# Woodenonez/DyObAv-MPCnWTA-Warehouse

Hardware: AMD Instinct MI355X
Metric: MPC solves/sec (N=20, batched) (higher is better)
Workload: dtype f32

## Files before the change

### dyobav-mpcnwta-warehouse_amd/csrc/nmpc_device.h

```cpp
#pragma once

#include <hip/hip_runtime.h>

#include "nmpc_sizes.h"
#include "wave_ops.h"

namespace nmpc {

#ifdef NMPC_PROFILE
constexpr int kProfSlots = 16;
#define NMPC_STAMP(I_, slot)                                              \
    do {                                                                  \
        __builtin_amdgcn_sched_barrier(0);                                \
        const unsigned long long t_ = __builtin_amdgcn_s_memtime();       \
        (I_).prof[slot] += t_ - (I_).t_last;                              \
        (I_).t_last = t_;                                                 \
        __builtin_amdgcn_sched_barrier(0);                                \
    } while (0)
#elif defined(NMPC_MARK)
constexpr int kProfSlots = 0;
#define NMPC_STAMP(I_, slot)                                                                      \
    do {                                                                                          \
        __builtin_amdgcn_sched_barrier(0);                                                        \
        if ((slot) < 7 || (slot) > 11) asm volatile("s_nop %0" : : "n"(8 + ((slot) & 7)));   \
// ... 106 lines not shown
__device__ __forceinline__ float tabs(float x) { return fabsf(x); }
__device__ __forceinline__ double tabs(double x) { return fabs(x); }
__device__ __forceinline__ float tpow(float x, float y) { return powf(x, y); }
__device__ __forceinline__ double tpow(double x, double y) { return pow(x, y); }
__device__ __forceinline__ float tmax(float a, float b) { return fmaxf(a, b); }
__device__ __forceinline__ double tmax(double a, double b) { return fmax(a, b); }
__device__ __forceinline__ float tmin(float a, float b) { return fminf(a, b); }
__device__ __forceinline__ double tmin(double a, double b) { return fmin(a, b); }
__device__ __forceinline__ bool tfinite(float x) { return isfinite(x); }
__device__ __forceinline__ bool tfinite(double x) { return isfinite(x); }
__device__ __forceinline__ void sincos_medium(const float x, float& s, float& c)
{
    auto K = [](unsigned bits) { return __builtin_bit_cast(float, bits); };
    const float ax = __builtin_fabsf(x);
    const float fn = __builtin_rintf(ax * K(0x3f22f983u));
    const int n = (int)fn;
    float r = __builtin_fmaf(fn, K(0xbfc90fdau), ax);
    r = __builtin_fmaf(fn, K(0xb3a22168u), r);
    r = __builtin_fmaf(fn, K(0xa7c234c4u), r);
    const float r2 = r * r;
    float t = __builtin_fmaf(r2, K(0xb94c1982u), K(0x3c0881c4u));
    t = __builtin_fmaf(r2, t, K(0xbe2aaa9du));
    t = r2 * t;
    const float sr = __builtin_fmaf(r, t, r);
    float u = __builtin_fmaf(r2, K(0x37d75334u), K(0xbab64f3bu));
    u = __builtin_fmaf(r2, u, K(0x3d2aabf7u));
    u = __builtin_fmaf(r2, u, K(0xbf000004u));
    const float cr = __builtin_fmaf(r2, u, 1.0f);
    const unsigned flip = ((unsigned)n << 30) & 0x80000000u;
    const bool odd = (n & 1) != 0;
    const unsigned sb = __builtin_bit_cast(unsigned, odd ? cr : sr) ^ flip ^
                        (__builtin_bit_cast(unsigned, x) & 0x80000000u);
    const unsigned cb = __builtin_bit_cast(unsigned, odd ? -sr : cr) ^ flip;
    s = __builtin_bit_cast(float, sb);
    c = __builtin_bit_cast(float, cb);
}
constexpr float kSincosMediumBound = 131072.0f;

template <typename T>
__device__ __forceinline__ T tclamp(T x, T lo, T hi)
{
    return tmin(tmax(x, lo), hi);
}
template <typename T>
__device__ __forceinline__ T ls_point(T u, T f, T d, T tau)
{
#pragma clang fp contract(off)
    const T a = (T(1) - tau) * f;
    const T b = tau * d;
    return (u - a) - b;
}

template <typename T>
struct Lim;
template <>
struct Lim<float> {
    static constexpr float min_pos = 1.17549435e-38f, eps = 1.1920929e-7f, big = 3.0e38f;
};
template <>
struct Lim<double> {
    static constexpr double min_pos = 2.2250738585072014e-308, eps = 2.220446049250313e-16, big = 1.0e300;
};

__device__ __forceinline__ double fast_rcp(double x)
{
    x = fmin(x, Lim<double>::big);
    double r = __builtin_amdgcn_rcp(x);
    r = __builtin_fma(__builtin_fma(-x, r, 1.0), r, r);
    r = __builtin_fma(__builtin_fma(-x, r, 1.0), r, r);
    return r;
}
__device__ __forceinline__ float fast_rcp(float x)
{
    x = fminf(x, Lim<float>::big);
    float r = __builtin_amdgcn_rcpf(x);
    r = __builtin_fmaf(__builtin_fmaf(-x, r, 1.0f), r, r);
    return r;
}

template <typename T>
struct alignas(16) Quad {
    T a, b, c, d;
};

template <typename T, int LPS, bool GLB = false, int RS = 0, bool COOP = false, bool HLP = false, bool AXIS = false>
struct Instance {
    static_assert(!AXIS || (RS > 0 && LPS == 3) || GLB, "axis-aligned variant: three-lane register table, or the compressed global table");
    static constexpr bool CMP = AXIS && GLB;
    static_assert(!(GLB && RS > 0), "the register-resident table replaces the LDS table, not the global one");
    static_assert(RS == 0 || LPS == 3 || LPS == 1, "register-resident table: three lanes or one lane per horizon step");
    const KParams<T>& kp;
    const T* __restrict__ p;
    T* lds;
    T* wsp;

    int lane, k, r;
    bool act, lead, tail;

    T rv_k, qstc_k, qdyn_k;

    int n_dyn, n_pad;
    int n_grp = 0;
    int n_poly;
    int n_fl0, n_flp;
    T wzero;

    int n_psi, n_grad;
    int cw_ = 0, CW_ = 1, xb = 0;
    T* coop_x = nullptr;
    __device__ __forceinline__ int cw() const { return COOP ? cw_ : 0; }
    __device__ __forceinline__ int CW() const { return COOP ? CW_ : 1; }
    __device__ __forceinline__ int reg_rows() const { return RS == 0 ? 0 : HLP ? 3 * CW() * (RS / 2) : LPS * CW() * RS; }
    T tab[RS > 0 ? RS : 1][9];
#ifdef NMPC_PROFILE
    unsigned long long* prof;
    unsigned long long t_last;
    unsigned int pcnt[3] = {0u, 0u, 0u};
    __device__ __forceinline__ unsigned long long prof_value(int i) const { return prof[i] + (!COOP && i >= 13 ? pcnt[i - 13] : 0u); }
#endif

    __device__ __forceinline__ Instance(const KParams<T>& kp_, const T* p_, T* lds_, T* ws_ = nullptr)
        : kp(kp_), p(p_), lds(lds_), wsp(ws_)
    {
        lane = threadIdx.x & 63;
        k = lane / LPS;
        r = lane - k * LPS;
        act = k < kp.N;
        lead = act && r == 0;
        tail = act && r == LPS - 1;
        n_psi = n_grad = 0;
#ifdef NMPC_PROFILE
        __shared__ unsigned long long prof_sh[8][kProfSlots];
        prof = prof_sh[(threadIdx.x >> 6) & 7];
        for (int i = 0; i < kProfSlots; ++i) prof[i] = 0;
        t_last = __builtin_amdgcn_s_memtime();
#endif
    }

    __device__ __forceinline__ int load()
    {
        const int N = kp.N, NP1 = kp.N + 1;
        const int kk = act ? k : 0;
        rv_k = p[kp.off_rv + kk];
        qstc_k = p[kp.off_qstc + kk];
        qdyn_k = p[kp.off_qdyn + kk];

        int* iflag = reinterpret_cast<int*>(lds + kp.lds_iflag);
        const unsigned lane_lt = __builtin_amdgcn_mbcnt_hi(~0u, __builtin_amdgcn_mbcnt_lo(~0u, 0u));
        (void)lane_lt;

        const int ne = kp.Ndyn * NP1;
        for (int j = lane; j < kp.Ndyn; j += 64) iflag[j] = 0;
        __syncthreads();
        for (int e = lane; e < ne; e += 64) {
            const T* s = p + kp.off_od + e * 6;
            const bool nz = s[0] != T(0) || s[1] != T(0) || s[2] != T(0) || s[3] != T(0) || s[4] != T(0) ||
                            s[5] != T(0);
            if (nz) iflag[e / NP1] = 1;
        }
        __syncthreads();
        int base = 0;
        for (int j0 = 0; j0 < kp.Ndyn; j0 += 64) {
            const int j = j0 + lane;
            const bool on = j < kp.Ndyn && iflag[j] != 0;
            const unsigned long long bal = __ballot(on);
            const int pos = base + __popcll(bal & ((1ull << lane) - 1ull));
            __syncthreads();
            if (j < kp.Ndyn) iflag[j] = on ? pos : -1;
            base += __popcll(bal);
        }
        n_dyn = base;
        n_pad = kp.Ndyn - base;
        __syncthreads();
        if (n_dyn > kp.dyn_cap) return 4;
        bool skew = false;
        auto offdiag = [](const T x) { return x != T(0) && x == x; };
        auto entry = [&](const T* s, const T marg, Quad<T>& qa, Quad<T>& qb) {
            const T rx = s[2], ry = s[3];
            T sa, ca;
            tsincos(s[4], sa, ca);
            const T exp_ = rx + T(1e-6), eyp = ry + T(1e-6), exm = rx + marg + T(1e-6), eym = ry + marg + T(1e-6);
            const T ixp = T(1) / (exp_ * exp_), iyp = T(1) / (eyp * eyp);
            const T ixm = T(1) / (exm * exm), iym = T(1) / (eym * eym);
            const T cc = ca * ca, ss = sa * sa, cs = ca * sa;
            qa = Quad<T>{s[0], s[1], cc * ixp + ss * iyp, cs * (ixp - iyp)};
            qb = Quad<T>{ss * ixp + cc * iyp, cc * ixm + ss * iym, cs * (ixm - iym), ss * ixm + cc * iym};
        };
        if (RS > 0) {
            int* jof = reinterpret_cast<int*>(lds + kp.lds_hist);
            for (int j = lane; j < kp.Ndyn; j += 64) {
                const int row = iflag[j];
                if (row < 0) continue;
                const T* s = p + kp.off_od + (size_t)j * NP1 * 6;
                Quad<T> qa, qb;
                entry(s, kp.vm + kp.sm, qa, qb);
                Quad<T>* q = reinterpret_cast<Quad<T>*>(lds + row * kEllStride);
// ... 146 lines not shown
            if (i < kp.Nstc) {
#pragma unroll
                for (int c = 0; c < 12; ++c) {
                    v[c] = p[kp.off_os + 12 * i + c];
                    nz = nz || v[c] != T(0);
                }
            }
            const unsigned long long bal = __ballot(nz);
            const int pos = base + __popcll(bal & ((1ull << lane) - 1ull));
            if (nz) {
#pragma unroll
                for (int c = 0; c < 12; ++c) lds[kp.lds_poly + 12 * pos + c] = v[c];
            }
            base += __popcll(bal);
        }
        n_poly = base;
        if (lane < 12 * LPS) lds[kp.lds_poly + 12 * n_poly + lane] = lane % 12 < 4 ? T(-1) : T(0);
        int* idx0 = reinterpret_cast<int*>(lds + kp.lds_fl0);
        int* idxp = reinterpret_cast<int*>(lds + kp.lds_fl);
        int b0 = 0, bp = 0;
        for (int j0 = 0; j0 < kp.Nother; j0 += 64) {
            const int j = j0 + lane;
            bool nz0 = false, nzp = false;
            if (j < kp.Nother) {
                nz0 = j >= 1 && (p[kp.off_c0 + 3 * j] != T(0) || p[kp.off_c0 + 3 * j + 1] != T(0));
                for (int kk = 0; kk < N; ++kk)
                    nzp = nzp || p[kp.off_c + 3 * (j * N + kk)] != T(0) || p[kp.off_c + 3 * (j * N + kk) + 1] != T(0);
            }
            const unsigned long long bal0 = __ballot(nz0), balp = __ballot(nzp);
            const unsigned long long lt = (1ull << lane) - 1ull;
            if (nz0) idx0[b0 + __popcll(bal0 & lt)] = j;
            if (nzp) idxp[bp + __popcll(balp & lt)] = j;
            b0 += __popcll(bal0);
            bp += __popcll(balp);
        }
        n_fl0 = b0;
        n_flp = bp;
        wzero = T(1000) * T(kp.Nother - 1 - b0) + T(10) * T(kp.Nother - bp);
        for (int i = lane; i < N; i += 64) {
            const int i2 = i + 1 < N ? i + 1 : N - 1;
            const T ax = p[kp.off_rs + 3 * i], ay = p[kp.off_rs + 3 * i + 1];
            const T dx = p[kp.off_rs + 3 * i2] - ax, dy = p[kp.off_rs + 3 * i2 + 1] - ay;
            T* q = lds + kp.lds_seg + 4 * i;
            q[0] = ax;
            q[1] = ay;
            q[2] = dx;
            q[3] = dy;
            lds[kp.lds_seginv + i] = T(1) / (dx * dx + dy * dy + T(1e-16));
        }
        for (int i = N + lane; i < seg_table_len(N); i += 64) {
            T* q = lds + kp.lds_seg + 4 * i;
            q[0] = T(1e15);
            q[1] = T(1e15);
            q[2] = T(0);
            q[3] = T(0);
            lds[kp.lds_seginv + i] = T(1);
        }
        __syncthreads();
        return 0;
    }

    typedef const T __attribute__((address_space(1))) * HotPtr;
    static __device__ __forceinline__ HotPtr hot_ptr(const T* q)
    {
        unsigned long long a = (unsigned long long)q;
        asm volatile("" : "+s"(a));
        return (HotPtr)a;
    }

    static __device__ __forceinline__ T pair_dot(T av, T aw, T bv, T bw)
    {
        if constexpr (sizeof(T) == 4) return __builtin_fmaf(aw, bw, av * bv);
        else return __builtin_fma(aw, bw, av * bv);
    }
    __device__ __forceinline__ T dot2(T av, T aw, T bv, T bw) const
    {
        return wave_sum(lead ? pair_dot(av, aw, bv, bw) : T(0));
    }
    __device__ __forceinline__ void dot2x2(T av, T aw, T bv, T bw, T cv, T cw, T dv, T dw, T& ab, T& cd) const
    {
        wave_sum2(lead ? pair_dot(av, aw, bv, bw) : T(0), lead ? pair_dot(cv, cw, dv, dw) : T(0), ab, cd);
    }

    template <bool GRAD, bool FLAT = false>
    __device__ __forceinline__ void eval(const T v, const T w, const T c, const T inv_cdiv, const T yv, const T yw,
                                         T& psi, T& f2sq_out, T& gv, T& gw)
    {
        const auto* kh = cold_args<T>();
        const int N = kh->N, NP1 = N + 1;
        const T ts = kh->ts, inv_ts = kh->inv_ts;
        constexpr bool HOIST = !COOP && RS > 0;
        const int o_poly_ = HOIST ? kh->lds_poly : 0, o_seg_ = HOIST ? kh->lds_seg : 0, o_seginv_ = HOIST ? kh->lds_seginv : 0,
                  o_left_ = HOIST ? kh->lds_left : 0;
        const T c_amin_ = HOIST ? kh->amin : T(0), c_amax_ = HOIST ? kh->amax : T(0), c_wamax_ = HOIST ? kh->wamax : T(0),
                c_safe2_ = HOIST ? kh->safe2 : T(0);
#define NMPC_COLD(field, local) (HOIST ? local : kh->field)
#define o_poly NMPC_COLD(lds_poly, o_poly_)
#define o_seg NMPC_COLD(lds_seg, o_seg_)
#define o_seginv NMPC_COLD(lds_seginv, o_seginv_)
#define o_left NMPC_COLD(lds_left, o_left_)
#define c_amin NMPC_COLD(amin, c_amin_)
#define c_amax NMPC_COLD(amax, c_amax_)
#define c_wamax NMPC_COLD(wamax, c_wamax_)
#define c_safe2 NMPC_COLD(safe2, c_safe2_)
        int k = this->k, r = this->r;
        asm volatile("" : "+v"(k), "+v"(r));
        const bool act = k < N, lead = act && r == 0, tail = act && r == LPS - 1;
        const T sixth = T(1.0 / 6.0);
        const HotPtr ph = hot_ptr(p);
        typedef const T __attribute__((address_space(4))) * HotScalarPtr;
        const HotScalarPtr phs = HOIST ? (HotScalarPtr)(unsigned long long)ph : nullptr;
        const T x0 = HOIST ? phs[2] : ph[2], y0 = HOIST ? phs[3] : ph[3], th0 = HOIST ? phs[4] : ph[4];
        const T vinit = ph[0], winit = ph[1], xg = ph[5], yg = ph[6], thg = ph[7];
        const T qvel = ph[8 + 1], rvw = ph[8 + 3], rww = ph[8 + 4], qN = ph[8 + 5], qthN = ph[8 + 6], qrpd = ph[8 + 7],
                accp = ph[8 + 8], waccp = ph[8 + 9];
        if (HOIST) asm volatile("" : : "s"(N), "s"(ts), "s"(inv_ts), "s"(o_poly_), "s"(o_seg_), "s"(o_seginv_), "s"(o_left_), "s"(c_amin_), "s"(c_amax_), "s"(c_wamax_), "s"(c_safe2_), "s"(x0), "s"(y0), "s"(th0));
        n_psi++;
        if (GRAD) n_grad++;
        NMPC_STAMP(*this, 0);
        constexpr bool BATCH = !COOP && RS > 6 && LPS == 3 && AXIS && !FLAT && sizeof(T) == 4;
        const bool batch = BATCH && N == 20;
        Quad<T> sgs[7];
        T invs[7];
        Quad<T> pol[2][3];
        if (batch) {
            const int i0 = act ? k + r : N;
            const Quad<T>* sp = reinterpret_cast<const Quad<T>*>(lds + o_seg) + i0;
            const T* ip = lds + o_seginv + i0;
#pragma unroll
            for (int j = 0; j < 7; ++j) {
                sgs[j] = sp[LPS * j];
                invs[j] = ip[LPS * j];
            }
            const Quad<T>* pq = reinterpret_cast<const Quad<T>*>(lds + o_poly) + 3 * r;
#pragma unroll
            for (int j = 0; j < 2; ++j)
#pragma unroll
                for (int q = 0; q < 3; ++q) pol[j][q] = pq[3 * LPS * j + q];
        }

        const T dth = ts * w;
        const T sc_th = wave_scan_incl(lead ? dth : T(0));
        const T th_k = th0 + wave_shift_up<LPS>(sc_th);
        const T th_n = th0 + sc_th;
        const T hh = dth * T(0.5);
        T s0, c0, sh, ch;
        if (sizeof(T) == 4 && __ballot(!(tabs(th_k) < T(kSincosMediumBound))) == 0ull) {
            float fs, fc;
            sincos_medium((float)th_k, fs, fc);
            s0 = (T)fs;
            c0 = (T)fc;
        } else {
            tsincos(th_k, s0, c0);
        }
        if (sizeof(T) == 4 && __ballot(!(tabs(hh) < T(0.785))) == 0ull) {
            const float r = (float)hh, r2 = r * r;
            auto K = [](unsigned bits) { return __builtin_bit_cast(float, bits); };
            float t = __builtin_fmaf(r2, K(0xb94c1982u), K(0x3c0881c4u));
            t = __builtin_fmaf(r2, t, K(0xbe2aaa9du));
            t = r2 * t;
            sh = (T)__builtin_fmaf(r, t, r);
            float u = __builtin_fmaf(r2, K(0x37d75334u), K(0xbab64f3bu));
            u = __builtin_fmaf(r2, u, K(0x3d2aabf7u));
            u = __builtin_fmaf(r2, u, K(0xbf000004u));
            ch = (T)__builtin_fmaf(r2, u, 1.0f);
        } else {
            tsincos(hh, sh, ch);
        }
        const T s2h = T(2) * sh * ch, c2h = T(1) - T(2) * sh * sh;
        const T s1 = s0 * ch + c0 * sh, c1 = c0 * ch - s0 * sh;
        const T s2 = s0 * c2h + c0 * s2h, c2 = c0 * c2h - s0 * s2h;
        const T Ck = (c0 + T(4) * c1 + c2) * sixth;
        const T Sk = (s0 + T(4) * s1 + s2) * sixth;
        T sX = lead ? ts * v * Ck : T(0), sY = lead ? ts * v * Sk : T(0);
        wave_scan_incl2(sX, sY);
        const T X = x0 + sX, Y = y0 + sY;

        NMPC_STAMP(*this, 1);
        T cst = 0, gx = 0, gy = 0;
        T Pp = 0, hpx = 0, hpy = 0;

        if (act) {
            int npl = n_poly;
            asm volatile("" : "+s"(npl));
            const int ptrips = (npl + LPS - 1) / LPS;
            const Quad<T>* pq = reinterpret_cast<const Quad<T>*>(lds + o_poly) + 3 * r;
            auto poly_terms = [&](const Quad<T>& b, const Quad<T>& a0, const Quad<T>& a1) {
                const T h0 = tmax(T(0), b.a - a0.a * X - a1.a * Y);
                const T h1 = tmax(T(0), b.b - a0.b * X - a1.b * Y);
                const T h2 = tmax(T(0), b.c - a0.c * X - a1.c * Y);
                const T h3 = tmax(T(0), b.d - a0.d * X - a1.d * Y);
                const T p01 = h0 * h1, p23 = h2 * h3, ind = p01 * p23;
                cst += qstc_k * ind * ind;
                Pp += ind;
                if (GRAD && __ballot(ind > T(0)) != 0ull) {
                    const T e0 = h1 * p23, e1 = h0 * p23, e2 = p01 * h3, e3 = p01 * h2;
                    T dix = -(a0.a * e0 + a0.b * e1 + a0.c * e2 + a0.d * e3);
                    T diy = -(a1.a * e0 + a1.b * e1 + a1.c * e2 + a1.d * e3);
                    if (!(ind > T(0))) {
// ... 910 lines not shown
template <typename T, typename Inst>
__device__ __forceinline__ void lbfgs_apply(const Inst& I, const Quad<T>* hist, const LaneVec<T>& rho, const int N,
                                            const int kk, const int mem_, const int lb_head, const int lb_active,
                                            const T lb_gamma, const T fv, const T fw, T& dv, T& dw)
{
    const int head = __builtin_amdgcn_readfirstlane(lb_head), nact = __builtin_amdgcn_readfirstlane(lb_active);
    const int mem = __builtin_amdgcn_readfirstlane(mem_);
    LaneVec<T> al;
    T qv = fv, qw = fw;
    int sl = head;
    const int NS = lbfgs_slot_stride(N);
    Quad<T> cur = hist[sl * NS + kk];
    for (int i = 0; i < nact; ++i) {
        int sn = sl + 1 == mem ? 0 : sl + 1;
        if (i + 1 >= nact) sn = sl;
        const Quad<T> nxt = hist[sn * NS + kk];
        const T a = rho.get(sl) * I.dot2(cur.a, cur.b, qv, qw);
        al.set(i, a);
        qv -= a * cur.c;
        qw -= a * cur.d;
        cur = nxt;
        sl = sn;
    }
    if (nact > 0) {
        qv *= lb_gamma;
        qw *= lb_gamma;
    }
    for (int j = 0; j < nact; ++j) {
        const int i = nact - 1 - j;
        const T beta = rho.get(sl) * I.dot2(cur.c, cur.d, qv, qw);
        const T ab = al.get(i) - beta;
        qv += ab * cur.a;
        qw += ab * cur.b;
        int sn = sl == 0 ? mem - 1 : sl - 1;
        if (j + 1 >= nact) sn = sl;
        cur = hist[sn * NS + kk];
        sl = sn;
    }
    dv = qv;
    dw = qw;
}

enum Phase : int { PH_LS, PH_LIP, PH_NOLS, PH_INIT_B, PH_INIT_A, PH_OUTER };

template <typename T, int LPS, bool GLB, int RS = 0, bool COOP = false, bool HLP = false, bool AXIS = false, bool TRACE = false>
__device__ __forceinline__ void solve_instance(const KParams<T>& kp, const int inst, T* lds)
{
    int tr_n = 0, tr_pair = -1;
    const int wave = COOP ? __builtin_amdgcn_readfirstlane((int)(threadIdx.x >> 6)) : 0;
    const T GAMMA_L = T(0.95), LIP_EPS_UPD = T(1e-6), MIN_L = T(1e-10), MAX_L = T(1e9);
    const int MAX_LIP = 10, MAX_LS = 10;

    Instance<T, LPS, GLB, RS, COOP, HLP, AXIS> I(kp, kp.P + (size_t)inst * kp.np, lds, GLB ? kp.ws + (long long)inst * kp.ws_stride : nullptr);
    if (COOP) {
        I.cw_ = wave;
        I.CW_ = (int)(blockDim.x >> 6);
        I.coop_x = lds + kp.lds_xch;
    }
    auto dyn_count = [&](int which) {
        if constexpr (!COOP && !TRACE) {
            int* const dc = cold_args<T>()->dyn_ctr;
            if (dc && threadIdx.x == 0) atomicAdd(dc + which, 1);
        }
    };
    dyn_count(0);
    if (const int bad = I.load()) {
        const T nan = __builtin_nanf("");
        const auto* kc = cold_args<T>();
        dyn_count(1);
        if (wave != 0) return;
        if (I.lead) {
            kc->U[(size_t)inst * 2 * kp.N + 2 * I.k] = nan;
            kc->U[(size_t)inst * 2 * kp.N + 2 * I.k + 1] = nan;
        }
        if (I.lane == 0) {
            if (kc->cost) kc->cost[inst] = nan;
            if (kc->status) kc->status[inst] = bad;
            if (kc->iters) kc->iters[2 * inst] = kc->iters[2 * inst + 1] = 0;
            if (kc->info)
                for (int i = 0; i < 8 + kProfSlots; ++i) kc->info[(size_t)inst * (8 + kProfSlots) + i] = 0;
        }
        return;
    }
    const int N = kp.N, n2 = kp.Ndyn;
    const int mem = kp.mem;
    const int kk = I.act ? I.k : 0;
    const bool lead = I.lead;
    const long long t_start = cold_args<T>()->time_budget > 0 ? (long long)__builtin_amdgcn_s_memrealtime() : 0;
    int cont_time = 1;
    int deep_slot = -1;

    T uv = 0, uw = 0, yv = 0, yw = 0;
    T c;
    {
        const auto* kc = cold_args<T>();
        if (kc->u0) {
            uv = kc->u0[(size_t)inst * 2 * N + 2 * kk];
            uw = kc->u0[(size_t)inst * 2 * N + 2 * kk + 1];
        }
        if (kc->y && kc->y_is_input) {
            yv = tclamp(kc->y[(size_t)inst * 2 * N + kk], T(-1e12), T(1e12));
            yw = tclamp(kc->y[(size_t)inst * 2 * N + N + kk], T(-1e12), T(1e12));
        }
        c = kc->c0v ? kc->c0v[inst] : kc->c_init;
    }
    if (!I.act) uv = uw = yv = yw = 0;
    const int resuming = __builtin_amdgcn_readfirstlane(cold_args<T>()->stage_in);

    T gv = 0, gw = 0, gpv = 0, gpw = 0;
    T hv = 0, hw = 0;
    T sv = 0, sw = 0;
    T dv = 0, dw = 0;
    T fv = 0, fw = 0;
    T pv = 0, pw = 0;
    T gamma = 0, inv_gamma = 0, L = 0, sigma = 0, tau = 1, cost_value = 0, norm_fpr = 0, rhs_ls = 0;
    T akkt_tol = cold_args<T>()->init_tol;
    int iteration = 0;
    Quad<T>* hist = reinterpret_cast<Quad<T>*>(lds + kp.lds_hist);
    LaneVec<T> rho;
    T osv = 0, osw = 0, ogv = 0, ogw = 0, lb_gamma = 1;
    int lb_active = 0, lb_head = 0;
    int lb_first = 1;
    T dyn = 0, dyn_plus = 0, f2n = 0, f2n_plus = 0;
    int alm_iter = 0, inner_total = 0, outer = 1, status = 0;
    int num_iter = 0, lip_it = 0, nls = 0;
    int cont = 1;
    T cost_half = 0, normh = 0, fbe_cur = 0;
    int fbe_valid = 0;

    const T vlo = kp.vmin, vhi = kp.vmax, wlo = -kp.wmax, whi = kp.wmax;
    auto project = [&](T& a, T& b) {
        a = tclamp(a, vlo, vhi);
        b = tclamp(b, wlo, whi);
    };
    auto grad_step_half = [&](T bv, T bw) {
        sv = bv - gamma * gv;
        sw = bw - gamma * gw;
        hv = sv;
        hw = sw;
        project(hv, hw);
    };
    auto reset_cache = [&]() {
        lb_active = 0;
        lb_first = true;
        rhs_ls = 0;
        tau = 1;
        L = 0;
        sigma = 0;
        cost_value = 0;
        iteration = 0;
        gamma = 0;
        inv_gamma = 0;
        fbe_valid = false;
    };

    auto park_ptr = [&](int buf) {
        return reinterpret_cast<Quad<T>*>(lds + kp.lds_park) + (COOP ? buf : wave) * (kParkQuads * 64) + I.lane;
    };
    auto park = [&]() {
        if (COOP && wave != 0) return;
        Quad<T>* const parkp = park_ptr(I.xb);
        parkp[0 * 64] = Quad<T>{osv, osw, ogv, ogw};
        parkp[1 * 64] = Quad<T>{gpv, gpw, sv, sw};
        parkp[2 * 64] = Quad<T>{pv, pw, dv, dw};
        parkp[3 * 64] = Quad<T>{hv, hw, fv, fw};
        parkp[4 * 64] = Quad<T>{uv, uw, gv, gw};
        asm volatile("" ::: "memory");
    };
    auto unpark = [&]() {
        asm volatile("" ::: "memory");
        const Quad<T>* const parkp = park_ptr(I.xb ^ 1);
        const Quad<T> q0 = parkp[0 * 64], q1 = parkp[1 * 64], q2 = parkp[2 * 64], q3 = parkp[3 * 64],
                      q4 = parkp[4 * 64];
        osv = q0.a, osw = q0.b, ogv = q0.c, ogw = q0.d;
        gpv = q1.a, gpw = q1.b, sv = q1.c, sw = q1.d;
        pv = q2.a, pw = q2.b, dv = q2.c, dw = q2.d;
        hv = q3.a, hw = q3.b, fv = q3.c, fw = q3.d;
        uv = q4.a, uw = q4.b, gv = q4.c, gw = q4.d;
    };

    if (resuming) {
        const T* rs = cold_args<T>()->resume + (size_t)inst * kResumeStride;
        uv = rs[0 * 64 + I.lane], uw = rs[1 * 64 + I.lane], yv = rs[2 * 64 + I.lane], yw = rs[3 * 64 + I.lane];
        gpv = rs[4 * 64 + I.lane], gpw = rs[5 * 64 + I.lane];
        const T* sc = rs + 6 * 64;
        c = sc[0];
        akkt_tol = sc[1];
        dyn = sc[2];
        f2n = sc[3];
        alm_iter = __builtin_amdgcn_readfirstlane((int)sc[4]);
        outer = __builtin_amdgcn_readfirstlane((int)sc[5]) + 1;
        inner_total = __builtin_amdgcn_readfirstlane((int)sc[6]);
        I.n_psi = __builtin_amdgcn_readfirstlane((int)sc[7]);
        I.n_grad = __builtin_amdgcn_readfirstlane((int)sc[8]);
        yv = tclamp(yv, T(-1e12), T(1e12));
        yw = tclamp(yw, T(-1e12), T(1e12));
    }
    int phase = PH_INIT_A;
    T ev = uv, ew = uw, ec = c;
    T inv_cdiv = T(1) / (c > T(1) ? c : T(1));
    int want_grad = 1;
    T r_psi = 0, r_f2 = 0, r_gv = 0, r_gw = 0;

    auto anyb = [](bool cond) { return __builtin_amdgcn_ballot_w64(cond) != 0ull; };
    for (;;) {
        const T e_icd = ec == c ? inv_cdiv : T(1);
#ifndef NMPC_NO_PARK
        park();
#endif
        constexpr bool kFlat = false;
        if (want_grad)
            I.template eval<true, kFlat>(ev, ew, ec, e_icd, yv, yw, r_psi, r_f2, r_gv, r_gw);
        else
            I.template eval<false, kFlat>(ev, ew, ec, e_icd, yv, yw, r_psi, r_f2, r_gv, r_gw);
#ifndef NMPC_NO_PARK
        unpark();
#endif

        bool step_head = false;
        bool step_done = false;

        if (phase == PH_LS) {
            NMPC_STAMP(I, 7);
            cost_value = r_psi;
            gv = r_gv;
            gw = r_gw;
            grad_step_half(pv, pw);
            const T t1 = sv - hv, t2 = sw - hw;
            T d2, gg;
            I.dot2x2(t1, t2, t1, t2, gv, gw, gv, gw, d2, gg);
            const T lhs = cost_value - T(0.5) * gamma * gg + T(0.5) * d2 * inv_gamma;
            fbe_cur = lhs;
            fbe_valid = true;
            NMPC_STAMP(I, 10);
            if (anyb(lhs > rhs_ls) && nls < MAX_LS) {
                tau *= T(0.5);
                nls++;
                pv = ls_point(uv, fv, dv, tau);
                pw = ls_point(uw, fw, dw, tau);
                ev = pv;
                ew = pw;
                ec = c;
                want_grad = true;
                continue;
            }
            uv = pv;
            uw = pw;
            step_done = true;
        } else if (phase == PH_LIP) {
            NMPC_STAMP(I, 7);
            cost_half = r_psi;
            const T ip = I.dot2(gv, gw, fv, fw);
            const T rhs = cost_value + LIP_EPS_UPD * tabs(cost_value) - ip +
                          (GAMMA_L * T(0.5) * inv_gamma) * (norm_fpr * norm_fpr);
            if (anyb(cost_half > rhs && L < MAX_L) && lip_it < MAX_LIP) {
                lb_active = 0;
                lb_first = true;
                L *= T(2);
                gamma *= T(0.5);
                inv_gamma *= T(2);
                fbe_valid = false;
                grad_step_half(uv, uw);
                fv = uv - hv;
                fw = uw - hw;
                norm_fpr = tsqrt(I.dot2(fv, fw, fv, fw));
                lip_it++;
                ev = hv;
                ew = hw;
                ec = c;
                want_grad = false;
                continue;
            }
            sigma = (T(1) - GAMMA_L) * T(0.25) * inv_gamma;
            if constexpr (TRACE) tr_pair = -1;
            if (lb_first) {
                lb_first = false;
                osv = uv;
                osw = uw;
                ogv = fv;
                ogw = fw;
            } else {
                const T nsv = uv - osv, nsw = uw - osw, nyv = fv - ogv, nyw = fw - ogw;
                T ys, ss;
                I.dot2x2(nsv, nsw, nyv, nyw, nsv, nsw, nsv, nsw, ys, ss);
                bool ok = true;
                const auto* kc = cold_args<T>();
                const T sy_eps = kc->sy_eps, cbfgs_eps = kc->cbfgs_eps, cbfgs_alpha = kc->cbfgs_alpha;
                if (ss <= Lim<T>::min_pos || (sy_eps > T(0) && ys <= sy_eps)) {
                    ok = false;
                } else if (cbfgs_eps > T(0) && cbfgs_alpha > T(0)) {
                    const T lhs = ys / ss;
                    const T rhs_c = cbfgs_eps * (cbfgs_alpha == T(1) ? norm_fpr : tpow(norm_fpr, cbfgs_alpha));
                    ok = lhs > rhs_c && tfinite(lhs) && tfinite(rhs_c);
                }
                ok = anyb(ok);
                if constexpr (TRACE) tr_pair = ok ? 1 : 0;
                if (ok) {
                    osv = uv;
                    osw = uw;
                    ogv = fv;
                    ogw = fw;
                    lb_head = lb_head == 0 ? mem - 1 : lb_head - 1;
                    if (lead) hist[lb_head * lbfgs_slot_stride(N) + I.k] = Quad<T>{nsv, nsw, nyv, nyw};
                    rho.set(lb_head, T(1) / ys);
                    lb_gamma = ys / I.dot2(nyv, nyw, nyv, nyw);
                    lb_active = lb_active + 1 < mem ? lb_active + 1 : mem;
                    __syncthreads();
                }
            }
            NMPC_STAMP(I, 8);
            if (iteration > 0) {
                lbfgs_apply(I, hist, rho, N, kk, mem, lb_head, lb_active, lb_gamma, fv, fw, dv, dw);
                NMPC_STAMP(I, 9);
                if (!fbe_valid) {
                    const T t1 = sv - hv, t2 = sw - hw;
                    T dist2, gg;
                    I.dot2x2(t1, t2, t1, t2, gv, gw, gv, gw, dist2, gg);
                    fbe_cur = cost_value - T(0.5) * gamma * gg + T(0.5) * dist2 * inv_gamma;
                }
                rhs_ls = fbe_cur - sigma * norm_fpr * norm_fpr;
                tau = 1;
                nls = 0;
                pv = ls_point(uv, fv, dv, tau);
                pw = ls_point(uw, fw, dw, tau);
                ev = pv;
                ew = pw;
                ec = c;
                want_grad = true;
                phase = PH_LS;
                continue;
            } else {
                uv = hv;
                uw = hw;
                ev = uv;
                ew = uw;
                ec = c;
                want_grad = true;
                phase = PH_NOLS;
                continue;
            }
        } else if (phase == PH_NOLS) {
            fbe_valid = false;
            cost_value = r_psi;
            gv = r_gv;
            gw = r_gw;
            grad_step_half(uv, uw);
            step_done = true;
        } else if (phase == PH_INIT_B) {
            const T d1 = r_gv - gv, d2 = r_gw - gw;
            L = tsqrt(I.dot2(d1, d2, d1, d2)) / normh;
            gamma = GAMMA_L / tmax(L, MIN_L);
            inv_gamma = T(1) / gamma;
            sigma = (T(1) - GAMMA_L) * T(0.25) * inv_gamma;
            cost_value = r_psi;
            grad_step_half(uv, uw);
            step_head = true;
        } else if (phase == PH_INIT_A) {
            cost_value = r_psi;
            gv = r_gv;
            gw = r_gw;
            const auto* kc = cold_args<T>();
            const T lip_eps = kc->lip_eps, lip_delta = kc->lip_delta;
            const T e1 = lip_eps * uv, e2 = lip_eps * uw;
            const T h1 = e1 > lip_delta ? e1 : lip_delta, h2 = e2 > lip_delta ? e2 : lip_delta;
            normh = tsqrt(I.dot2(h1, h2, h1, h2));
            if (I.act) {
                uv += h1;
                uw += h2;
            }
            ev = uv;
            ew = uw;
            ec = c;
            want_grad = true;
            phase = PH_INIT_B;
            continue;
        } else {
            const auto* kc = cold_args<T>();
            const T f_u = r_psi;
            f2n_plus = tsqrt(r_f2);
            const T v_up = wave_shift_up<LPS>(uv), w_up = wave_shift_up<LPS>(uw);
            const T vprev = I.k == 0 ? I.p[0] : v_up;
            const T wprev = I.k == 0 ? I.p[1] : w_up;
            const T acc = (uv - vprev) * kc->inv_ts, wacc = (uw - wprev) * kc->inv_ts;
            const T za = acc + yv / c, zw = wacc + yw / c;
            T ypv = yv + c * (acc - tclamp(za, kc->amin, kc->amax));
            T ypw = yw + c * (wacc - tclamp(zw, -kc->wamax, kc->wamax));
            if (!I.act) ypv = ypw = 0;
            const T e1 = ypv - yv, e2 = ypw - yw;
            dyn_plus = tsqrt(I.dot2(e1, e2, e1, e2));
            const T SMALL = Lim<T>::eps;
            const int single = kc->single_inner;
            const bool c1 = single || (alm_iter > 0 && dyn_plus <= c * kc->delta_tol + SMALL);
            const bool c2 = n2 == 0 || f2n_plus <= kc->delta_tol + SMALL;
            const bool c3 = akkt_tol <= kc->tol + SMALL;
            bool finished = false, converged = false, out_of_time = false;
            if (anyb(c1 && c2 && c3) && (!single || status == 0)) {
                finished = converged = true;
            } else {
                const bool stall = alm_iter == 0 || anyb((dyn_plus <= kc->suff_dec * dyn + SMALL) &&
                                                         (n2 == 0 || f2n_plus <= kc->suff_dec * f2n + SMALL));
                if (!stall && !single) {
                    c *= kc->pen_update;
                    inv_cdiv = T(1) / (c > T(1) ? c : T(1));
                }
                akkt_tol = tmax(akkt_tol * kc->tol_update, kc->tol);
                alm_iter++;
                dyn = dyn_plus;
                f2n = f2n_plus;
                if (!single) {
                    yv = ypv;
                    yw = ypw;
                }
                reset_cache();
                const int me = kc->max_evals;
                if (outer >= kc->max_outer) finished = true;
                else if (!cont_time || (me > 0 && I.n_psi >= me)) {
                    finished = true;
                    out_of_time = true;
                }
            }
            if (finished) {
                if (!converged) status = (out_of_time || status == 2) ? 2 : 1;
                bool finite = tfinite(uv) && tfinite(uw) && tfinite(f_u);
                if (__ballot(!finite) != 0ull) status = 3;
                dyn_count(1);
                if (wave != 0) return;
                int ri = inst;
                asm volatile("" : "+s"(ri));
                if (lead) {
                    kc->U[(size_t)ri * 2 * N + 2 * I.k] = uv;
                    kc->U[(size_t)ri * 2 * N + 2 * I.k + 1] = uw;
                    if (kc->y) {
                        kc->y[(size_t)ri * 2 * N + I.k] = yv;
                        kc->y[(size_t)ri * 2 * N + N + I.k] = yw;
                    }
                }
                if constexpr (TRACE)
                    if (I.lane == 0 && kc->trace) kc->trace[0] = T(tr_n < kc->trace_cap ? tr_n : kc->trace_cap);
                if (I.lane == 0) {
                    if (kc->cost) kc->cost[ri] = f_u;
                    if (kc->status) kc->status[ri] = status;
                    if (kc->iters) {
                        kc->iters[2 * ri] = outer;
                        kc->iters[2 * ri + 1] = inner_total;
                    }
                    if (kc->info) {
                        T* o = kc->info + (size_t)ri * (8 + kProfSlots);
                        o[0] = norm_fpr;
                        o[1] = f2n_plus;
                        o[2] = dyn_plus;
                        o[3] = c;
                        o[4] = T(I.n_psi);
                        o[5] = T(I.n_grad);
                        o[6] = 0;
                        o[7] = COOP ? T(-I.CW()) : T(0);
#ifdef NMPC_PROFILE
                        for (int i = 0; i < kProfSlots; ++i) o[8 + i] = T(I.prof_value(i));
#endif
                    }
                }
                return;
            }
            {
                const int cap = kc->stage_outer_cap;
                bool park_now = cap > 0 && outer >= cap;
                if constexpr (!COOP && !TRACE) {
                    int* const dc = kc->dyn_ctr;
                    if (!park_now && dc) {
                        const int total = __hip_atomic_load(dc + 2, __ATOMIC_RELAXED, __HIP_MEMORY_SCOPE_AGENT);
                        const int started = __hip_atomic_load(dc + 0, __ATOMIC_RELAXED, __HIP_MEMORY_SCOPE_AGENT);
                        const int gone = __hip_atomic_load(dc + 1, __ATOMIC_RELAXED, __HIP_MEMORY_SCOPE_AGENT);
                        park_now = __builtin_amdgcn_readfirstlane((started >= total && total - gone <= kc->dyn_park) ? 1 : 0) != 0;
                    }
                }
                if (park_now) {
                    dyn_count(1);
                    if (wave != 0) return;
                    int ri = inst;
                    asm volatile("" : "+s"(ri));
                    T* rs = kc->resume + (size_t)ri * kResumeStride;
                    rs[0 * 64 + I.lane] = uv, rs[1 * 64 + I.lane] = uw, rs[2 * 64 + I.lane] = yv, rs[3 * 64 + I.lane] = yw;
                    rs[4 * 64 + I.lane] = gpv, rs[5 * 64 + I.lane] = gpw;
                    if (I.lane == 0) {
                        T* sc = rs + 6 * 64;
                        sc[0] = c;
                        sc[1] = akkt_tol;
                        sc[2] = dyn;
                        sc[3] = f2n;
                        sc[4] = T(alm_iter);
                        sc[5] = T(outer);
                        sc[6] = T(inner_total);
                        sc[7] = T(I.n_psi);
                        sc[8] = T(I.n_grad);
                        sc[9] = T(0);
                        sc[10] = T(0);
                        kc->status[ri] = -1;
                    }
                    return;
                }
            }
            ev = uv;
            ew = uw;
            ec = c;
            want_grad = true;
            phase = PH_INIT_A;
            num_iter = 0;
            cont = true;
            outer++;
            yv = tclamp(yv, T(-1e12), T(1e12));
            yw = tclamp(yw, T(-1e12), T(1e12));
            continue;
        }

        if (step_done) {
            if constexpr (TRACE) {
                const auto* kc = cold_args<T>();
                if (kc->trace && tr_n < kc->trace_cap && wave == 0) {
                    T* t = kc->trace + (size_t)(tr_n + 1) * kTraceHead + (size_t)tr_n * 2 * N;
                    if (I.lane == 0) {
                        t[0] = T(outer), t[1] = T(iteration), t[2] = T(lip_it), t[3] = T(iteration == 0 ? 0 : nls);
                        t[4] = T(tr_pair), t[5] = T(lb_active), t[6] = gamma, t[7] = norm_fpr, t[8] = cost_value;
                        t[9] = iteration == 0 ? T(0) : tau, t[10] = T(I.n_psi), t[11] = T(I.n_grad), t[12] = 0, t[13] = 0;
                        t[14] = c, t[15] = 0;
                    }
                    if (lead) {
                        t[kTraceHead + 2 * I.k] = uv;
                        t[kTraceHead + 2 * I.k + 1] = uw;
                    }
                }
                tr_n++;
            }
            iteration++;
            if (!cont || !cont_time) {
                step_head = false;
            } else {
                num_iter++;
                const auto* kc = cold_args<T>();
                cont = num_iter < kc->max_inner;
                const long long budget = kc->time_budget;
                if (budget > 0) cont_time = (long long)__builtin_amdgcn_s_memrealtime() - t_start <= budget;
                const int me = kc->max_evals;
                if (me > 0 && I.n_psi >= me) cont_time = 0;
                step_head = true;
                if constexpr (!COOP && !TRACE) {
                    int* const dc = kc->dyn_ctr;
                    if ((num_iter & 15) == 0 && dc && kc->deep) {
                        const int total = __hip_atomic_load(dc + 2, __ATOMIC_RELAXED, __HIP_MEMORY_SCOPE_AGENT);
                        const int started = __hip_atomic_load(dc + 0, __ATOMIC_RELAXED, __HIP_MEMORY_SCOPE_AGENT);
                        const int gone = __hip_atomic_load(dc + 1, __ATOMIC_RELAXED, __HIP_MEMORY_SCOPE_AGENT);
                        if (__builtin_amdgcn_readfirstlane((started >= total && total - gone <= kc->dyn_park) ? 1 : 0)) {
                            int slot = 0;
                            if (I.lane == 0) slot = atomicAdd(dc + 3, 1);
                            slot = __builtin_amdgcn_readfirstlane(slot);
                            if (slot < kc->deep_slots) {
                                deep_slot = slot;
                                break;
                            }
                        }
                    }
                }
            }
        }

        bool inner_exit = !step_head;
        if (step_head) {
            if (iteration >= 1) {
                gpv = gv;
                gpw = gw;
            }
            fv = uv - hv;
            fw = uw - hw;
            const T a1 = fv + gamma * (gv - gpv), a2 = fw + gamma * (gw - gpw);
            T ff, aa;
            I.dot2x2(fv, fw, fv, fw, a1, a2, a1, a2, ff, aa);
            norm_fpr = tsqrt(ff);
            const auto* kc = cold_args<T>();
            const T akkt = kc->akkt_form ? tsqrt(aa) * inv_gamma : tsqrt(aa);
            NMPC_STAMP(I, 11);
            if (anyb(norm_fpr < kc->tol && akkt < akkt_tol)) {
                inner_exit = true;
            } else {
                lip_it = 0;
                ev = hv;
                ew = hw;
                ec = c;
                want_grad = false;
                phase = PH_LIP;
                continue;
            }
        }
        if (inner_exit) {
            status = !cont ? 1 : !cont_time ? 2 : 0;
            inner_total += num_iter;
            uv = hv;
            uw = hw;
            ev = uv;
            ew = uw;
            ec = T(0);
            want_grad = false;
            phase = PH_OUTER;
            continue;
        }
    }
    if constexpr (!COOP && !TRACE) {
        const auto* kc = cold_args<T>();
        const int slot = deep_slot;
    park();
    T* const dsc = lds + kc->lds_deepsc;
    if (I.lane == 0) {
        dsc[kDeepScGamma] = gamma, dsc[kDeepScInvGamma] = inv_gamma, dsc[kDeepScL] = L, dsc[kDeepScCost] = cost_value;
        dsc[kDeepScFbe] = fbe_cur, dsc[kDeepScAkkt] = akkt_tol, dsc[kDeepScC] = c, dsc[kDeepScLbGamma] = lb_gamma;
        dsc[kDeepScDyn] = dyn, dsc[kDeepScF2n] = f2n;
        dsc[kDeepScIteration] = T(iteration), dsc[kDeepScNumIter] = T(num_iter), dsc[kDeepScCont] = T(cont);
        dsc[kDeepScContTime] = T(cont_time), dsc[kDeepScFbeValid] = T(fbe_valid), dsc[kDeepScLbActive] = T(lb_active);
        dsc[kDeepScLbHead] = T(lb_head), dsc[kDeepScLbFirst] = T(lb_first), dsc[kDeepScAlmIter] = T(alm_iter);
        dsc[kDeepScInnerTotal] = T(inner_total), dsc[kDeepScOuter] = T(outer), dsc[kDeepScNPsi] = T(I.n_psi);
        dsc[kDeepScNGrad] = T(I.n_grad);
    }
    T* g = kc->deep + (size_t)slot * deep_park_stride(N);
    const T* src = reinterpret_cast<const T*>(park_ptr(I.xb)) - 4 * I.lane;
    for (int i = I.lane; i < kParkQuads * 64 * 4; i += 64) g[i] = src[i];
    g += kParkQuads * 64 * 4;
    const int nr = deep_ring_elems(N);
    const T* ring = reinterpret_cast<const T*>(hist);
    for (int i = I.lane; i < nr; i += 64) g[i] = ring[i];
    g += nr;
    g[I.lane] = yv, g[64 + I.lane] = yw, g[128 + I.lane] = rho.v;
    if (I.lane < kDeepScalars) g[192 + I.lane] = dsc[I.lane];
    int ri = inst;
    asm volatile("" : "+s"(ri));
    if (I.lane == 0) {
        T* sc = kc->resume + (size_t)ri * kResumeStride + 6 * 64;
        sc[3] = f2n;
        sc[7] = T(I.n_psi);
        sc[10] = T(slot + 1);
        kc->status[ri] = -1;
    }

        dyn_count(1);
    }
}

}
```

Before: 68970.

## Keep solver vectors homed in LDS and bank scalar constants in one VGPR

Adds a lane-indexed constant bank: cold scalar parameters and x0/y0/th0 are packed one per lane into a single VGPR and read back with read_lane, so they no longer occupy SGPRs or need reloads from the constant buffer inside eval. Solver vectors (u, g, h, f, s, gp, p, d, os, og) now live in an LDS park area. Each phase loads only the halves it needs and stores updates right away, replacing the full park/unpark around every evaluation. The intent is to cut register pressure and the LDS traffic of the full spill on each eval. The cost is extra lane reads and scattered LDS accesses, plus correctness risk in tracking which homed values are still live.

```diff
diff --git a/dyobav-mpcnwta-warehouse_amd/csrc/nmpc_device.h b/dyobav-mpcnwta-warehouse_amd/csrc/nmpc_device.h
--- a/dyobav-mpcnwta-warehouse_amd/csrc/nmpc_device.h
+++ b/dyobav-mpcnwta-warehouse_amd/csrc/nmpc_device.h
@@ -212,6 +212,10 @@
 struct alignas(16) Quad {
     T a, b, c, d;
 };
+template <typename T>
+struct alignas(2 * sizeof(T)) Duo {
+    T a, b;
+};
 
 template <typename T, int LPS, bool GLB = false, int RS = 0, bool COOP = false, bool HLP = false, bool AXIS = false>
 struct Instance {
@@ -242,6 +246,41 @@
     __device__ __forceinline__ int CW() const { return COOP ? CW_ : 1; }
     __device__ __forceinline__ int reg_rows() const { return RS == 0 ? 0 : HLP ? 3 * CW() * (RS / 2) : LPS * CW() * RS; }
     T tab[RS > 0 ? RS : 1][9];
+    static constexpr bool BANK = !COOP && sizeof(T) == 4 && LPS == 3 && (RS == 4 || (RS == 14 && AXIS));
+    enum : int { kBkN, kBkPoly, kBkSeg, kBkSegInv, kBkLeft, kBkMaxInner, kBkMaxEvals, kBkAkktForm,
+                 kBkTs, kBkInvTs, kBkAmin, kBkAmax, kBkWamax, kBkSafe2, kBkX0, kBkY0, kBkTh0, kBkTol, kBkSyEps, kBkCbfgsEps,
+                 kBkCbfgsAlpha, kBkCount };
+    static_assert(kBkCount <= 64, "one entry per lane");
+    T cbank = 0;
+    __device__ __forceinline__ void bank_set(int i, T x) { cbank = lane == i ? x : cbank; }
+    __device__ __forceinline__ void bank_seti(int i, int x)
+    {
+        if constexpr (sizeof(T) == 4) bank_set(i, __builtin_bit_cast(T, x));
+    }
+    __device__ __forceinline__ T bank_f(int i) const { return read_lane(cbank, i); }
+    __device__ __forceinline__ int bank_i(int i) const
+    {
+        if constexpr (sizeof(T) == 4) return __builtin_bit_cast(int, read_lane(cbank, i));
+        else return 0;
+    }
+    __device__ __forceinline__ void bank_fence()
+    {
+        if constexpr (BANK) asm volatile("" : "+v"(cbank));
+    }
+    __device__ __forceinline__ void bank_fill()
+    {
+        if constexpr (BANK) {
+            const auto* kc = cold_args<T>();
+            bank_seti(kBkN, kc->N), bank_seti(kBkPoly, kc->lds_poly), bank_seti(kBkSeg, kc->lds_seg);
+            bank_seti(kBkSegInv, kc->lds_seginv), bank_seti(kBkLeft, kc->lds_left), bank_seti(kBkMaxInner, kc->max_inner);
+            bank_seti(kBkMaxEvals, kc->max_evals), bank_seti(kBkAkktForm, kc->akkt_form);
+            bank_set(kBkTs, kc->ts), bank_set(kBkInvTs, kc->inv_ts), bank_set(kBkAmin, kc->amin), bank_set(kBkAmax, kc->amax);
+            bank_set(kBkWamax, kc->wamax), bank_set(kBkSafe2, kc->safe2);
+            bank_set(kBkX0, p[2]), bank_set(kBkY0, p[3]), bank_set(kBkTh0, p[4]);
+            bank_set(kBkTol, kc->tol), bank_set(kBkSyEps, kc->sy_eps), bank_set(kBkCbfgsEps, kc->cbfgs_eps);
+            bank_set(kBkCbfgsAlpha, kc->cbfgs_alpha);
+        }
+    }
 #ifdef NMPC_PROFILE
     unsigned long long* prof;
     unsigned long long t_last;
@@ -554,18 +593,20 @@
         wave_sum2(lead ? pair_dot(av, aw, bv, bw) : T(0), lead ? pair_dot(cv, cw, dv, dw) : T(0), ab, cd);
     }
 
-    template <bool GRAD, bool FLAT = false>
+    template <bool GRAD, bool FLAT = false, bool BANKED = false>
     __device__ __forceinline__ void eval(const T v, const T w, const T c, const T inv_cdiv, const T yv, const T yw,
                                          T& psi, T& f2sq_out, T& gv, T& gw)
     {
+        constexpr bool BK = BANKED && BANK;
+        if constexpr (BK) bank_fence();
         const auto* kh = cold_args<T>();
-        const int N = kh->N, NP1 = N + 1;
-        const T ts = kh->ts, inv_ts = kh->inv_ts;
+        const int N = BK ? bank_i(kBkN) : kh->N, NP1 = N + 1;
+        const T ts = BK ? bank_f(kBkTs) : kh->ts, inv_ts = BK ? bank_f(kBkInvTs) : kh->inv_ts;
         constexpr bool HOIST = !COOP && RS > 0;
-        const int o_poly_ = HOIST ? kh->lds_poly : 0, o_seg_ = HOIST ? kh->lds_seg : 0, o_seginv_ = HOIST ? kh->lds_seginv : 0,
-                  o_left_ = HOIST ? kh->lds_left : 0;
-        const T c_amin_ = HOIST ? kh->amin : T(0), c_amax_ = HOIST ? kh->amax : T(0), c_wamax_ = HOIST ? kh->wamax : T(0),
-                c_safe2_ = HOIST ? kh->safe2 : T(0);
+        const int o_poly_ = BK ? bank_i(kBkPoly) : HOIST ? kh->lds_poly : 0, o_seg_ = BK ? bank_i(kBkSeg) : HOIST ? kh->lds_seg : 0,
+                  o_seginv_ = BK ? bank_i(kBkSegInv) : HOIST ? kh->lds_seginv : 0, o_left_ = BK ? bank_i(kBkLeft) : HOIST ? kh->lds_left : 0;
+        const T c_amin_ = BK ? bank_f(kBkAmin) : HOIST ? kh->amin : T(0), c_amax_ = BK ? bank_f(kBkAmax) : HOIST ? kh->amax : T(0),
+                c_wamax_ = BK ? bank_f(kBkWamax) : HOIST ? kh->wamax : T(0), c_safe2_ = BK ? bank_f(kBkSafe2) : HOIST ? kh->safe2 : T(0);
 #define NMPC_COLD(field, local) (HOIST ? local : kh->field)
 #define o_poly NMPC_COLD(lds_poly, o_poly_)
 #define o_seg NMPC_COLD(lds_seg, o_seg_)
@@ -582,11 +623,12 @@
         const HotPtr ph = hot_ptr(p);
         typedef const T __attribute__((address_space(4))) * HotScalarPtr;
         const HotScalarPtr phs = HOIST ? (HotScalarPtr)(unsigned long long)ph : nullptr;
-        const T x0 = HOIST ? phs[2] : ph[2], y0 = HOIST ? phs[3] : ph[3], th0 = HOIST ? phs[4] : ph[4];
+        const T x0 = BK ? bank_f(kBkX0) : HOIST ? phs[2] : ph[2], y0 = BK ? bank_f(kBkY0) : HOIST ? phs[3] : ph[3],
+                th0 = BK ? bank_f(kBkTh0) : HOIST ? phs[4] : ph[4];
         const T vinit = ph[0], winit = ph[1], xg = ph[5], yg = ph[6], thg = ph[7];
         const T qvel = ph[8 + 1], rvw = ph[8 + 3], rww = ph[8 + 4], qN = ph[8 + 5], qthN = ph[8 + 6], qrpd = ph[8 + 7],
                 accp = ph[8 + 8], waccp = ph[8 + 9];
-        if (HOIST) asm volatile("" : : "s"(N), "s"(ts), "s"(inv_ts), "s"(o_poly_), "s"(o_seg_), "s"(o_seginv_), "s"(o_left_), "s"(c_amin_), "s"(c_amax_), "s"(c_wamax_), "s"(c_safe2_), "s"(x0), "s"(y0), "s"(th0));
+        if (HOIST && !BK) asm volatile("" : : "s"(N), "s"(ts), "s"(inv_ts), "s"(o_poly_), "s"(o_seg_), "s"(o_seginv_), "s"(o_left_), "s"(c_amin_), "s"(c_amax_), "s"(c_wamax_), "s"(c_safe2_), "s"(x0), "s"(y0), "s"(th0));
         n_psi++;
         if (GRAD) n_grad++;
         NMPC_STAMP(*this, 0);
@@ -1663,6 +1705,8 @@
         }
         return;
     }
+    I.bank_fill();
+    constexpr bool BK = decltype(I)::BANK;
     const int N = kp.N, n2 = kp.Ndyn;
     const int mem = kp.mem;
     const int kk = I.act ? I.k : 0;
@@ -1735,6 +1779,11 @@
         fbe_valid = false;
     };
 
+#ifdef NMPC_NO_PARK
+    constexpr bool HOME = false;
+#else
+    constexpr bool HOME = !COOP && !TRACE && sizeof(T) == 4 && !(RS == 6 && !AXIS);
+#endif
     auto park_ptr = [&](int buf) {
         return reinterpret_cast<Quad<T>*>(lds + kp.lds_park) + (COOP ? buf : wave) * (kParkQuads * 64) + I.lane;
     };
@@ -1759,6 +1808,28 @@
         hv = q3.a, hw = q3.b, fv = q3.c, fw = q3.d;
         uv = q4.a, uw = q4.b, gv = q4.c, gw = q4.d;
     };
+    enum : int { kHomeOsOg, kHomeGpS, kHomePD, kHomeHF, kHomeUG };
+    auto ld_quad = [&](int q, T& a, T& b, T& c, T& d) {
+        if constexpr (HOME) {
+            const Quad<T> x = park_ptr(0)[q * 64];
+            a = x.a, b = x.b, c = x.c, d = x.d;
+        }
+    };
+    auto ld_half = [&](int q, int hi, T& a, T& b) {
+        if constexpr (HOME) {
+            const Duo<T> x = reinterpret_cast<const Duo<T>*>(park_ptr(0) + q * 64)[hi];
+            a = x.a, b = x.b;
+        }
+    };
+    auto ld_stay = [&]() {
+        if constexpr (HOME) asm volatile("" ::: "memory");
+    };
+    auto st_quad = [&](int q, T a, T b, T c, T d) {
+        if constexpr (HOME) park_ptr(0)[q * 64] = Quad<T>{a, b, c, d};
+    };
+    auto st_half = [&](int q, int hi, T a, T b) {
+        if constexpr (HOME) reinterpret_cast<Duo<T>*>(park_ptr(0) + q * 64)[hi] = Duo<T>{a, b};
+    };
 
     if (resuming) {
         const T* rs = cold_args<T>()->resume + (size_t)inst * kResumeStride;
@@ -1784,25 +1855,39 @@
     T r_psi = 0, r_f2 = 0, r_gv = 0, r_gw = 0;
 
     auto anyb = [](bool cond) { return __builtin_amdgcn_ballot_w64(cond) != 0ull; };
+    if constexpr (HOME) park();
     for (;;) {
         const T e_icd = ec == c ? inv_cdiv : T(1);
 #ifndef NMPC_NO_PARK
-        park();
+        if constexpr (!HOME) park();
 #endif
+        if constexpr (HOME) asm volatile("" ::: "memory");
         constexpr bool kFlat = false;
         if (want_grad)
-            I.template eval<true, kFlat>(ev, ew, ec, e_icd, yv, yw, r_psi, r_f2, r_gv, r_gw);
+            I.template eval<true, kFlat, true>(ev, ew, ec, e_icd, yv, yw, r_psi, r_f2, r_gv, r_gw);
         else
-            I.template eval<false, kFlat>(ev, ew, ec, e_icd, yv, yw, r_psi, r_f2, r_gv, r_gw);
+            I.template eval<false, kFlat, true>(ev, ew, ec, e_icd, yv, yw, r_psi, r_f2, r_gv, r_gw);
 #ifndef NMPC_NO_PARK
-        unpark();
+        if constexpr (!HOME) unpark();
 #endif
+        if constexpr (HOME) {
+            asm volatile("" ::: "memory");
+            osv = osw = ogv = ogw = gpv = gpw = sv = sw = pv = pw = dv = dw = hv = hw = fv = fw = uv = uw = gv = gw = 0;
+        }
 
         bool step_head = false;
         bool step_done = false;
 
         if (phase == PH_LS) {
             NMPC_STAMP(I, 7);
+            T cuv = uv, cuw = uw, cfv = fv, cfw = fw, cdv = dv, cdw = dw;
+            if constexpr (HOME) {
+                pv = ev, pw = ew;
+                ld_half(kHomeUG, 0, cuv, cuw);
+                ld_half(kHomeHF, 1, cfv, cfw);
+                ld_half(kHomePD, 1, cdv, cdw);
+                ld_stay();
+            }
             cost_value = r_psi;
             gv = r_gv;
             gw = r_gw;
@@ -1817,8 +1902,8 @@
             if (anyb(lhs > rhs_ls) && nls < MAX_LS) {
                 tau *= T(0.5);
                 nls++;
-                pv = ls_point(uv, fv, dv, tau);
-                pw = ls_point(uw, fw, dw, tau);
+                pv = ls_point(cuv, cfv, cdv, tau);
+                pw = ls_point(cuw, cfw, cdw, tau);
                 ev = pv;
                 ew = pw;
                 ec = c;
@@ -1827,9 +1912,17 @@
             }
             uv = pv;
             uw = pw;
+            st_half(kHomePD, 0, pv, pw);
             step_done = true;
         } else if (phase == PH_LIP) {
             NMPC_STAMP(I, 7);
+            if constexpr (HOME) {
+                hv = ev, hw = ew;
+                ld_quad(kHomeUG, uv, uw, gv, gw);
+                ld_half(kHomeHF, 1, fv, fw);
+                ld_quad(kHomeOsOg, osv, osw, ogv, ogw);
+                ld_stay();
+            }
             cost_half = r_psi;
             const T ip = I.dot2(gv, gw, fv, fw);
             const T rhs = cost_value + LIP_EPS_UPD * tabs(cost_value) - ip +
@@ -1844,6 +1937,8 @@
                 grad_step_half(uv, uw);
                 fv = uv - hv;
                 fw = uw - hw;
+                st_half(kHomeGpS, 1, sv, sw);
+                st_quad(kHomeHF, hv, hw, fv, fw);
                 norm_fpr = tsqrt(I.dot2(fv, fw, fv, fw));
                 lip_it++;
                 ev = hv;
@@ -1860,13 +1955,15 @@
                 osw = uw;
                 ogv = fv;
                 ogw = fw;
+                st_quad(kHomeOsOg, osv, osw, ogv, ogw);
             } else {
                 const T nsv = uv - osv, nsw = uw - osw, nyv = fv - ogv, nyw = fw - ogw;
                 T ys, ss;
                 I.dot2x2(nsv, nsw, nyv, nyw, nsv, nsw, nsv, nsw, ys, ss);
                 bool ok = true;
                 const auto* kc = cold_args<T>();
-                const T sy_eps = kc->sy_eps, cbfgs_eps = kc->cbfgs_eps, cbfgs_alpha = kc->cbfgs_alpha;
+                const T sy_eps = BK ? I.bank_f(I.kBkSyEps) : kc->sy_eps, cbfgs_eps = BK ? I.bank_f(I.kBkCbfgsEps) : kc->cbfgs_eps,
+                        cbfgs_alpha = BK ? I.bank_f(I.kBkCbfgsAlpha) : kc->cbfgs_alpha;
                 if (ss <= Lim<T>::min_pos || (sy_eps > T(0) && ys <= sy_eps)) {
                     ok = false;
                 } else if (cbfgs_eps > T(0) && cbfgs_alpha > T(0)) {
@@ -1881,6 +1978,7 @@
                     osw = uw;
                     ogv = fv;
                     ogw = fw;
+                    st_quad(kHomeOsOg, osv, osw, ogv, ogw);
                     lb_head = lb_head == 0 ? mem - 1 : lb_head - 1;
                     if (lead) hist[lb_head * lbfgs_slot_stride(N) + I.k] = Quad<T>{nsv, nsw, nyv, nyw};
                     rho.set(lb_head, T(1) / ys);
@@ -1892,8 +1990,10 @@
             NMPC_STAMP(I, 8);
             if (iteration > 0) {
                 lbfgs_apply(I, hist, rho, N, kk, mem, lb_head, lb_active, lb_gamma, fv, fw, dv, dw);
+                st_half(kHomePD, 1, dv, dw);
                 NMPC_STAMP(I, 9);
                 if (!fbe_valid) {
+                    ld_half(kHomeGpS, 1, sv, sw);
                     const T t1 = sv - hv, t2 = sw - hw;
                     T dist2, gg;
                     I.dot2x2(t1, t2, t1, t2, gv, gw, gv, gw, dist2, gg);
@@ -1913,6 +2013,7 @@
             } else {
                 uv = hv;
                 uw = hw;
+                st_half(kHomeUG, 0, uv, uw);
                 ev = uv;
                 ew = uw;
                 ec = c;
@@ -1921,6 +2022,7 @@
                 continue;
             }
         } else if (phase == PH_NOLS) {
+            if constexpr (HOME) uv = ev, uw = ew;
             fbe_valid = false;
             cost_value = r_psi;
             gv = r_gv;
@@ -1928,6 +2030,10 @@
             grad_step_half(uv, uw);
             step_done = true;
         } else if (phase == PH_INIT_B) {
+            if constexpr (HOME) {
+                uv = ev, uw = ew;
+                ld_half(kHomeUG, 1, gv, gw);
+            }
             const T d1 = r_gv - gv, d2 = r_gw - gw;
             L = tsqrt(I.dot2(d1, d2, d1, d2)) / normh;
             gamma = GAMMA_L / tmax(L, MIN_L);
@@ -1937,6 +2043,7 @@
             grad_step_half(uv, uw);
             step_head = true;
         } else if (phase == PH_INIT_A) {
+            if constexpr (HOME) uv = ev, uw = ew;
             cost_value = r_psi;
             gv = r_gv;
             gw = r_gw;
@@ -1949,6 +2056,7 @@
                 uv += h1;
                 uw += h2;
             }
+            st_quad(kHomeUG, uv, uw, gv, gw);
             ev = uv;
             ew = uw;
             ec = c;
@@ -1957,6 +2065,7 @@
             continue;
         } else {
             const auto* kc = cold_args<T>();
+            if constexpr (HOME) uv = ev, uw = ew;
             const T f_u = r_psi;
             f2n_plus = tsqrt(r_f2);
             const T v_up = wave_shift_up<LPS>(uv), w_up = wave_shift_up<LPS>(uw);
@@ -2060,6 +2169,7 @@
                     int ri = inst;
                     asm volatile("" : "+s"(ri));
                     T* rs = kc->resume + (size_t)ri * kResumeStride;
+                    ld_half(kHomeGpS, 0, gpv, gpw);
                     rs[0 * 64 + I.lane] = uv, rs[1 * 64 + I.lane] = uw, rs[2 * 64 + I.lane] = yv, rs[3 * 64 + I.lane] = yw;
                     rs[4 * 64 + I.lane] = gpv, rs[5 * 64 + I.lane] = gpw;
                     if (I.lane == 0) {
@@ -2117,10 +2227,10 @@
             } else {
                 num_iter++;
                 const auto* kc = cold_args<T>();
-                cont = num_iter < kc->max_inner;
+                cont = num_iter < (BK ? I.bank_i(I.kBkMaxInner) : kc->max_inner);
                 const long long budget = kc->time_budget;
                 if (budget > 0) cont_time = (long long)__builtin_amdgcn_s_memrealtime() - t_start <= budget;
-                const int me = kc->max_evals;
+                const int me = BK ? I.bank_i(I.kBkMaxEvals) : kc->max_evals;
                 if (me > 0 && I.n_psi >= me) cont_time = 0;
                 step_head = true;
                 if constexpr (!COOP && !TRACE) {
@@ -2148,20 +2258,25 @@
             if (iteration >= 1) {
                 gpv = gv;
                 gpw = gw;
+            } else {
+                ld_half(kHomeGpS, 0, gpv, gpw);
             }
             fv = uv - hv;
             fw = uw - hw;
+            st_quad(kHomeGpS, gpv, gpw, sv, sw);
+            st_quad(kHomeHF, hv, hw, fv, fw);
             const T a1 = fv + gamma * (gv - gpv), a2 = fw + gamma * (gw - gpw);
             T ff, aa;
             I.dot2x2(fv, fw, fv, fw, a1, a2, a1, a2, ff, aa);
             norm_fpr = tsqrt(ff);
             const auto* kc = cold_args<T>();
-            const T akkt = kc->akkt_form ? tsqrt(aa) * inv_gamma : tsqrt(aa);
+            const T akkt = (BK ? I.bank_i(I.kBkAkktForm) : kc->akkt_form) ? tsqrt(aa) * inv_gamma : tsqrt(aa);
             NMPC_STAMP(I, 11);
-            if (anyb(norm_fpr < kc->tol && akkt < akkt_tol)) {
+            if (anyb(norm_fpr < (BK ? I.bank_f(I.kBkTol) : kc->tol) && akkt < akkt_tol)) {
                 inner_exit = true;
             } else {
                 lip_it = 0;
+                st_quad(kHomeUG, uv, uw, gv, gw);
                 ev = hv;
                 ew = hw;
                 ec = c;
@@ -2175,6 +2290,7 @@
             inner_total += num_iter;
             uv = hv;
             uw = hw;
+            st_quad(kHomeUG, uv, uw, gv, gw);
             ev = uv;
             ew = uw;
             ec = T(0);
@@ -2186,7 +2302,13 @@
     if constexpr (!COOP && !TRACE) {
         const auto* kc = cold_args<T>();
         const int slot = deep_slot;
-    park();
+    if constexpr (HOME) {
+        st_quad(kHomeUG, uv, uw, gv, gw);
+        st_half(kHomeGpS, 1, sv, sw);
+        st_half(kHomeHF, 0, hv, hw);
+    } else {
+        park();
+    }
     T* const dsc = lds + kc->lds_deepsc;
     if (I.lane == 0) {
         dsc[kDeepScGamma] = gamma, dsc[kDeepScInvGamma] = inv_gamma, dsc[kDeepScL] = L, dsc[kDeepScCost] = cost_value;
```

Result: faster. 69920, median of 6 (+1.4%).
